# kelaendi/mused

Hardware: AMD Instinct MI355X
Metric: stream rows/sec, d=1024 l=128 window=10k synthetic (SWFD + kNN similarity + eigenstep + labels) (higher is better)
Workload: dtype f64; 1 GPU; synthetic d=1024 l=128 window=10000 k=50 (BASELINE config 2); stream=blob, W=10000, d=1024, l=128, k=50, modalities=1, swfd_levels=14, rccl_ranks=1, lanes_per_gpu=20, padded_window_slots=2

## Files before the change

### mused_amd/csrc/gemm_f64.h

```cpp
#pragma once
#include <cstdlib>
#include <mutex>
#include <type_traits>
#include "internal.h"

namespace mused {

typedef double v4f64 __attribute__((ext_vector_type(4)));

constexpr int GEMM_BM = 128;
constexpr int GEMM_BN = 128;
constexpr int GEMM_BK = 16;
constexpr int GEMM_LD = 144;
constexpr int GEMM_THREADS = 256;
constexpr int GEMM_LDS_BYTES = 2  * 2  * GEMM_BK * GEMM_LD * 8;

struct GemmArgs {
  const void* A;
  const void* B;
  long lda, ldb;
  long strideA, strideB;
  int M, N, K;
  int kchunk;
  int splitk;
  int bsplit;
  int tiles_m, tiles_n;
  const int* rep;
  const int* list;
  const int* kact;
  int sym;
  const double* tail;
  long tail_stride;
  int tail_per;
  const int* tail_split;
  int tail_split_stride;
  int tail_pend;
  const double* tail_zero;
};

struct GemmSplit {
  const double* tail;
  const double* zero;
  int nk, nend;
};
__device__ __forceinline__ const double* split_row(const double* __restrict__ base, long ld, const GemmSplit& sp, int r, int nrows,
                                                   bool& zero) {
  zero = r >= sp.nend || r >= nrows;
  return zero ? sp.zero : (r < sp.nk ? base + (long)r * ld : sp.tail + (long)(r - sp.nk) * ld);
}

template <typename TIn, bool VEC>
__device__ __forceinline__ void stage_load_kc(const TIn* __restrict__ src, long ld, int r0, int nrows, int k0,
                                              int kend, TIn (&r)[8]) {
  const int m = threadIdx.x & 127;
  const int kh = threadIdx.x >> 7;
  const int row = r0 + m;
  const int k = k0 + kh * 8;
  if (row < nrows) {
    const TIn* p = src + (long)row * ld + k;
    if (VEC && k + 8 <= kend) {
      if (sizeof(TIn) == 4) {
        const float4 a = *reinterpret_cast<const float4*>(p);
        const float4 b = *reinterpret_cast<const float4*>(p + 4);
        r[0] = a.x; r[1] = a.y; r[2] = a.z; r[3] = a.w;
        r[4] = b.x; r[5] = b.y; r[6] = b.z; r[7] = b.w;
      } else {
        const double2* q = reinterpret_cast<const double2*>(p);
#pragma unroll
        for (int j = 0; j < 4; ++j) {
          const double2 v = q[j];
// ... 361 lines not shown
    diag_mirror_groups<W, GI + 1>(g, epi, z, m0, patch, acc);
  }
}

template <int W, int N, typename Epi>
__device__ __forceinline__ void diag_store_blocks(const GemmArgs& g, const Epi& epi, int z, int m0, const v4f64 (&acc)[9]) {
  if constexpr (N < 9) {
    const int lane = threadIdx.x & 63;
    const int col = m0 + DIAG_J[W][N] * 16 + (lane & 15);
#pragma unroll
    for (int r = 0; r < 4; ++r) {
      const int row = m0 + DIAG_I[W][N] * 16 + (lane >> 4) + 4 * r;
      if (row < g.M && col < g.N) epi(z, row, col, acc[N][r]);
    }
    diag_store_blocks<W, N + 1>(g, epi, z, m0, acc);
  }
}

template <int W, typename Epi>
__device__ __forceinline__ void diag_epilogue(const GemmArgs& g, const Epi& epi, int z, int m0, double* smem,
                                              const v4f64 (&acc)[9]) {
  diag_store_blocks<W, 0>(g, epi, z, m0, acc);
  diag_mirror_groups<W, 0>(g, epi, z, m0, smem + W * (16 * DIAG_PATCH_LD), acc);
}

inline int gemm_sym_diag_enabled() {
  static const int on = [] {
    const char* s = getenv("MUSED_GEMM_SYM_DIAG");
    return (s && s[0] == '0') ? 0 : 1;
  }();
  return on;
}

template <typename TA, typename TB, bool A_KC, bool B_KC, bool VEC, typename Epi, bool TAIL = false>
__global__ __launch_bounds__(GEMM_THREADS, 2) void gemm_f64_kernel(GemmArgs g, Epi epi) {
  extern __shared__ __attribute__((aligned(16))) double smem[];

  int z = blockIdx.z;
  int zb = g.bsplit ? z / g.bsplit : z;
  if (g.list) {
    if (zb >= g.list[0]) return;
    const int e = g.list[1 + zb];
    z += (e - zb) * (g.bsplit ? g.bsplit : 1);
    zb = e;
  } else if (g.rep && g.rep[zb] != zb) return;
  int tm, tn;
  if (g.sym) {
    const int t = g.tiles_n, nwg = t * (t + 1) / 2;
    const int e = xcd_remap(blockIdx.x, nwg);
    int r = (int)((2.0 * t + 1.0 - sqrt((2.0 * t + 1.0) * (2.0 * t + 1.0) - 8.0 * e)) * 0.5);
    r = r < 0 ? 0 : (r > t - 1 ? t - 1 : r);
    while (r > 0 && r * t - r * (r - 1) / 2 > e) --r;
    while (r + 1 < t && (r + 1) * t - (r + 1) * r / 2 <= e) ++r;
    tm = r;
    tn = r + (e - (r * t - r * (r - 1) / 2));
  } else {
    const int nwg = g.tiles_m * g.tiles_n;
    const int wg = xcd_remap(blockIdx.x, nwg);
    constexpr int GROUP_M = 8;
    const int per_group = GROUP_M * g.tiles_n;
    const int group_id = wg / per_group;
    const int first_m = group_id * GROUP_M;
    const int group_size = min(g.tiles_m - first_m, GROUP_M);
    tm = first_m + (wg % group_size);
    tn = (wg % per_group) / group_size;
  }
  const int m0 = tm * GEMM_BM, n0 = tn * GEMM_BN;
  const bool mirror = g.sym && tm != tn;

  int k_lo = 0, k_hi = g.K;
  const TA* A = reinterpret_cast<const TA*>(g.A);
  const TB* B = reinterpret_cast<const TB*>(g.B);
  if (g.splitk) {
    k_lo = z * g.kchunk;
    k_hi = min(g.K, k_lo + g.kchunk);
  } else {
    A += (long)zb * g.strideA;
    B += (long)zb * g.strideB;
    if (g.bsplit) {
      k_lo = (z - zb * g.bsplit) * g.kchunk;
      k_hi = min(g.K, k_lo + g.kchunk);
    } else if (g.kact) {
      k_hi = min(g.K, g.kact[zb]);
    }
  }

  GemmSplit sp{};
  if constexpr (TAIL) {
    sp.nk = g.tail_split[(long)zb * g.tail_split_stride];
    sp.nend = sp.nk + g.tail_pend;
    sp.tail = g.tail + (long)(zb / g.tail_per) * g.tail_stride;
    sp.zero = g.tail_zero;
  }

  if constexpr (std::is_same<TA, TB>::value && A_KC == B_KC) {
    if (g.sym == 2 && tm == tn) {
      const int w = __builtin_amdgcn_readfirstlane(threadIdx.x >> 6);
      v4f64 acc9[9];
      gemm_tile_mainloop_diag<TA, A_KC, VEC, TAIL>(g, A, m0, k_lo, k_hi, smem, w, acc9, sp);
      switch (w) {
        case 0: diag_epilogue<0>(g, epi, z, m0, smem, acc9); break;
        case 1: diag_epilogue<1>(g, epi, z, m0, smem, acc9); break;
        case 2: diag_epilogue<2>(g, epi, z, m0, smem, acc9); break;
        default: diag_epilogue<3>(g, epi, z, m0, smem, acc9); break;
      }
      return;
    }
  }

  const int lane = threadIdx.x & 63;
  const int wave = threadIdx.x >> 6;
  const int wr = wave >> 1, wc = wave & 1;
  const int kq = lane >> 4, li = lane & 15;

  v4f64 acc[4][4];
  gemm_tile_mainloop<TA, TB, A_KC, B_KC, VEC, TAIL>(g, A, B, m0, n0, k_lo, k_hi, smem, acc, sp);

#pragma unroll
  for (int i = 0; i < 4; ++i) {
#pragma unroll
    for (int j = 0; j < 4; ++j) {
      const int col = n0 + wc * 64 + j * 16 + li;
#pragma unroll
      for (int r = 0; r < 4; ++r) {
        const int row = m0 + wr * 64 + i * 16 + kq + 4 * r;
// ... 13 lines not shown
          const int j = half * 2 + jj;
          const int col = n0 + wc * 64 + j * 16 + li;
#pragma unroll
          for (int r = 0; r < 4; ++r) {
            const int rl = i * 16 + kq + 4 * r;
            const int rg = m0 + wr * 64 + rl;
            patch[(jj * 16 + li) * 65 + rl] = (rg < g.M && col < g.N) ? epi.value(col, rg, acc[i][j][r]) : 0.0;
          }
        }
      const int rowm = m0 + wr * 64 + lane;
#pragma unroll 8
      for (int c = 0; c < 32; ++c) {
        const int colm = n0 + wc * 64 + half * 32 + c;
        if (colm < g.N && rowm < g.M) epi.put(z, colm, rowm, patch[c * 65 + lane]);
      }
    }
  }
}

struct EpiStore {
  double* C;
  long ldc;
  long strideC;
  double alpha;
  __device__ __forceinline__ void operator()(int z, int row, int col, double v) const {
    C[(long)z * strideC + (long)row * ldc + col] = alpha * v;
  }
  __device__ __forceinline__ double value(int, int, double v) const { return alpha * v; }
  __device__ __forceinline__ void put(int z, int row, int col, double val) const {
    C[(long)z * strideC + (long)row * ldc + col] = val;
  }
};

template <typename TA, typename TB, bool A_KC, bool B_KC, bool VEC, typename Epi, bool TAIL = false>
int gemm_f64_prepare_t() {
  static LdsOptIn opt;
  auto k = gemm_f64_kernel<TA, TB, A_KC, B_KC, VEC, Epi, TAIL>;
  const hipError_t err = allow_dynamic_lds(opt, reinterpret_cast<const void*>(k), GEMM_LDS_BYTES);
  MUSED_CHECK_HIP(err);
  return MUSED_OK;
}

template <typename TA, typename TB, bool A_KC, bool B_KC, typename Epi, bool TAIL = false>
int gemm_f64_launch_t(GemmArgs g, int batch, Epi epi, bool vec, hipStream_t stream) {
  g.tiles_m = cdiv(g.M, GEMM_BM);
  g.tiles_n = cdiv(g.N, GEMM_BN);
  if (g.sym) g.sym = (g.sym != 3 && gemm_sym_diag_enabled()) ? 2 : 1;
  if (g.M <= 0 || g.N <= 0 || batch <= 0) return MUSED_OK;
  dim3 grid(g.sym ? g.tiles_n * (g.tiles_n + 1) / 2 : g.tiles_m * g.tiles_n, 1, batch);
  int rc;
  if (vec) {
    if ((rc = gemm_f64_prepare_t<TA, TB, A_KC, B_KC, true, Epi, TAIL>())) return rc;
    hipLaunchKernelGGL((gemm_f64_kernel<TA, TB, A_KC, B_KC, true, Epi, TAIL>), grid, dim3(GEMM_THREADS), GEMM_LDS_BYTES,
                       stream, g, epi);
  } else {
    if ((rc = gemm_f64_prepare_t<TA, TB, A_KC, B_KC, false, Epi, TAIL>())) return rc;
    hipLaunchKernelGGL((gemm_f64_kernel<TA, TB, A_KC, B_KC, false, Epi, TAIL>), grid, dim3(GEMM_THREADS), GEMM_LDS_BYTES,
                       stream, g, epi);
  }
  MUSED_LAUNCH_CHECK();
  return MUSED_OK;
}

template <typename T>
static inline bool vec_ok(const void* p, long ld, long stride) {
  const long e = 16 / (long)sizeof(T);
  return ((uintptr_t)p % 16 == 0) && (ld % e == 0) && (stride % e == 0);
}

}
```

### mused_amd/csrc/gemm_f64.hip

```cpp
#include <stdarg.h>

#include "gemm_f64.h"
#include "internal.h"

namespace mused {

static thread_local char g_err[512] = "";

void set_error(const char* fmt, ...) {
  va_list ap;
  va_start(ap, fmt);
  vsnprintf(g_err, sizeof(g_err), fmt, ap);
  va_end(ap);
}

const char* last_error() { return g_err; }

int gemm_f64_prepare_all() {
  int rc = 0;
#define PREP(a, b, v) rc |= gemm_f64_prepare_t<double, double, a, b, v, EpiStore>()
  PREP(true, true, true); PREP(true, true, false); PREP(true, false, true); PREP(true, false, false);
  PREP(false, true, true); PREP(false, true, false); PREP(false, false, true); PREP(false, false, false);
#undef PREP
#define PREP(a, b, v) rc |= gemm_f64_prepare_t<double, double, a, b, v, EpiStore, true>()
  PREP(true, true, true); PREP(true, true, false); PREP(true, false, true); PREP(true, false, false);
#undef PREP
  return rc ? MUSED_ERR_HIP : MUSED_OK;
}

static int gemm_set_tail(GemmArgs& g, const GemmTail& t, bool a_kc, bool b_kc, long ld, bool& vec) {
  MUSED_REQUIRE(t.rows && t.split && t.zero_row && t.per_lane >= 1 && t.pend >= 0, "gemm_f64: bad tail");
  MUSED_REQUIRE(a_kc && (!b_kc || g.sym), "gemm_f64: a tail needs a Gram launch or a K-rows operand B");
  g.tail = t.rows; g.tail_stride = t.lane_stride; g.tail_per = t.per_lane;
  g.tail_split = t.split; g.tail_split_stride = t.split_stride; g.tail_pend = t.pend; g.tail_zero = t.zero_row;
  if (g.sym && t.plain_diag) g.sym = 3;
  vec = vec && vec_ok<double>(t.rows, ld, t.lane_stride) && vec_ok<double>(t.zero_row, ld, 0);
  return MUSED_OK;
}

int gemm_f64(bool a_kc, bool b_kc, const double* A, long lda, long strideA, const double* B, long ldb,
             long strideB, double* C, long ldc, long strideC, int M, int N, int K, int batch, double alpha,
             hipStream_t stream, const int* rep, const int* list, const int* kact, const GemmTail* tail) {
  GemmArgs g;
  memset(&g, 0, sizeof(g));
  g.A = A; g.B = B; g.lda = lda; g.ldb = ldb; g.strideA = strideA; g.strideB = strideB;
  g.M = M; g.N = N; g.K = K; g.splitk = 0; g.kchunk = 0;
  g.rep = rep; g.list = list; g.kact = kact;
  g.sym = (A == B && a_kc == b_kc && lda == ldb && strideA == strideB && M == N) ? 1 : 0;
  EpiStore epi{C, ldc, strideC, alpha};
  bool vec = vec_ok<double>(A, lda, strideA) && vec_ok<double>(B, ldb, strideB);
  if (tail) {
    int rc;
    if ((rc = gemm_set_tail(g, *tail, a_kc, b_kc, ldb, vec))) return rc;
    if (b_kc) return gemm_f64_launch_t<double, double, true, true, EpiStore, true>(g, batch, epi, vec, stream);
    return gemm_f64_launch_t<double, double, true, false, EpiStore, true>(g, batch, epi, vec, stream);
  }
  if (a_kc && b_kc) return gemm_f64_launch_t<double, double, true, true>(g, batch, epi, vec, stream);
  if (a_kc && !b_kc) return gemm_f64_launch_t<double, double, true, false>(g, batch, epi, vec, stream);
  if (!a_kc && b_kc) return gemm_f64_launch_t<double, double, false, true>(g, batch, epi, vec, stream);
  return gemm_f64_launch_t<double, double, false, false>(g, batch, epi, vec, stream);
}

int gemm_f64_splitk(bool a_kc, bool b_kc, const double* A, long lda, const double* B, long ldb, double* partial,
                    int M, int N, int K, int kchunk, int nsplit, hipStream_t stream) {
  MUSED_REQUIRE(kchunk > 0 && kchunk % GEMM_BK == 0 && nsplit >= 1 && (long)kchunk * nsplit >= K,
                "gemm_f64_splitk: bad kchunk %d x %d for K=%d", kchunk, nsplit, K);
  GemmArgs g;
  memset(&g, 0, sizeof(g));
  g.A = A; g.B = B; g.lda = lda; g.ldb = ldb;
  g.M = M; g.N = N; g.K = K; g.splitk = 1; g.kchunk = kchunk;
  EpiStore epi{partial, (long)N, (long)M * N, 1.0};
  const bool vec = vec_ok<double>(A, lda, 0) && vec_ok<double>(B, ldb, 0);
  if (a_kc && b_kc) return gemm_f64_launch_t<double, double, true, true>(g, nsplit, epi, vec, stream);
  if (a_kc && !b_kc) return gemm_f64_launch_t<double, double, true, false>(g, nsplit, epi, vec, stream);
  if (!a_kc && b_kc) return gemm_f64_launch_t<double, double, false, true>(g, nsplit, epi, vec, stream);
  return gemm_f64_launch_t<double, double, false, false>(g, nsplit, epi, vec, stream);
}

__global__ void splitk_reduce_kernel(const double* __restrict__ partial, int nsplit, long count,
                                     double* __restrict__ out) {
  const long i = (long)blockIdx.x * blockDim.x + threadIdx.x;
  if (i >= count) return;
  double s = 0.0;
  for (int z = 0; z < nsplit; ++z) s += partial[(long)z * count + i];
  out[i] = s;
}

int gemm_f64_batched_splitk(bool a_kc, bool b_kc, const double* A, long lda, long strideA, const double* B, long ldb, long strideB,
                            double* partial, int M, int N, int K, int batch, int kchunk, int nsplit, hipStream_t stream,
                            const int* rep, const int* list, const GemmTail* tail) {
  MUSED_REQUIRE(kchunk > 0 && kchunk % GEMM_BK == 0 && nsplit >= 1 && (long)kchunk * nsplit >= K,
                "gemm_f64_batched_splitk: bad kchunk %d x %d for K=%d", kchunk, nsplit, K);
  GemmArgs g;
// ... 75 lines not shown

int mused_gemm_f64_batched_rep(int a_kc, int b_kc, const double* A, long lda, long strideA, const double* B, long ldb,
                               long strideB, double* C, long ldc, long strideC, int M, int N, int K, int batch,
                               double alpha, const int* rep, void* stream) {
  return mused::gemm_f64(a_kc != 0, b_kc != 0, A, lda, strideA, B, ldb, strideB, C, ldc, strideC, M, N, K, batch,
                         alpha, (hipStream_t)stream, rep);
}

int mused_debug_gemm_f64_batched_active(int a_kc, int b_kc, const double* A, long lda, long strideA, const double* B, long ldb,
                                        long strideB, double* C, long ldc, long strideC, int M, int N, int K, int batch,
                                        double alpha, const int* list, const int* kact, void* stream) {
  return mused::gemm_f64(a_kc != 0, b_kc != 0, A, lda, strideA, B, ldb, strideB, C, ldc, strideC, M, N, K, batch,
                         alpha, (hipStream_t)stream, nullptr, list, kact);
}

int mused_debug_gemm_f64_batched_tail(int a_kc, int b_kc, const double* A, long lda, long strideA, const double* B, long ldb,
                                      long strideB, double* C, long ldc, long strideC, int M, int N, int K, int batch,
                                      const int* list, const int* kact, const double* tail, long tail_stride, int per_lane,
                                      const int* split, int split_stride, int pend, const double* zero_row, int plain_diag, double* partial,
                                      int kchunk,
                                      int nsplit, void* stream) {
  MUSED_REQUIRE(A && B && C && tail && split && batch >= 1, "mused_debug_gemm_f64_batched_tail: bad arguments");
  const mused::GemmTail t{tail, tail_stride, per_lane, split, split_stride, pend, zero_row, plain_diag};
  if (nsplit <= 1)
    return mused::gemm_f64(a_kc != 0, b_kc != 0, A, lda, strideA, B, ldb, strideB, C, ldc, strideC, M, N, K, batch, 1.0,
                           (hipStream_t)stream, nullptr, list, kact, &t);
  MUSED_REQUIRE(partial && ldc == N && strideC == (long)M * N, "mused_debug_gemm_f64_batched_tail: split-K writes a dense C");
  int rc = mused::gemm_f64_batched_splitk(a_kc != 0, b_kc != 0, A, lda, strideA, B, ldb, strideB, partial, M, N, K, batch, kchunk,
                                          nsplit, (hipStream_t)stream, nullptr, list, &t);
  if (rc != MUSED_OK) return rc;
  return mused::gemm_batched_splitk_reduce(partial, nsplit, (long)M * N, C, batch, nullptr, (hipStream_t)stream, list);
}

int mused_gemm_f64_splitk(int a_kc, int b_kc, const double* A, long lda, const double* B, long ldb, double* partial,
                          double* C, int M, int N, int K, int kchunk, int nsplit, void* stream) {
  MUSED_REQUIRE(A && B && partial && C && M >= 0 && N >= 0 && K >= 0, "mused_gemm_f64_splitk: bad arguments");
  int rc = mused::gemm_f64_splitk(a_kc != 0, b_kc != 0, A, lda, B, ldb, partial, M, N, K, kchunk, nsplit,
                                  (hipStream_t)stream);
  if (rc != MUSED_OK || M == 0 || N == 0) return rc;
  return mused::gemm_splitk_reduce(partial, nsplit, (long)M * N, C, (hipStream_t)stream);
}

int mused_gemm_f64_batched_splitk(int a_kc, int b_kc, const double* A, long lda, long strideA, const double* B, long ldb,
                                  long strideB, double* partial, double* C, int M, int N, int K, int batch, int kchunk,
                                  int nsplit, const int* rep, void* stream) {
  MUSED_REQUIRE(A && B && partial && C && M >= 0 && N >= 0 && K >= 0 && batch >= 1,
                "mused_gemm_f64_batched_splitk: bad arguments");
  int rc = mused::gemm_f64_batched_splitk(a_kc != 0, b_kc != 0, A, lda, strideA, B, ldb, strideB, partial, M, N, K, batch,
                                          kchunk, nsplit, (hipStream_t)stream, rep);
  if (rc != MUSED_OK || M == 0 || N == 0) return rc;
  return mused::gemm_batched_splitk_reduce(partial, nsplit, (long)M * N, C, batch, rep, (hipStream_t)stream);
}

}
```

### mused_amd/csrc/internal.h

```cpp
#pragma once
#include "common.h"

#include <atomic>
#include <mutex>

extern "C" int mused_row_sq_norms(const void* X, int dtype, long n, int d, long ld, double* out, void* stream);

namespace mused {

int select_from_records(const double* rec, int n, int kind, int k, int* out_idx, unsigned long long* out_mask,
                        int mask_words, hipStream_t stream);
int select_from_tag_sets(const int* rowptr, const int* tags, const int* postptr, const int* postrow, int n, int k,
                         int* out_idx, unsigned long long* out_mask, int mask_words, hipStream_t stream);
int select_max_fused_rows(bool tag_sets);
int select_window_records(const double* rec, const int* vrank, int s, int e, int kind, int k, unsigned long long* out_mask,
                          int mask_words, hipStream_t stream);
int select_window_tag_sets(const int* rowptr, const int* tags, const int* postptr, const int* postrow, const int* vrank, int s,
                           int e, int k, unsigned long long* out_mask, int mask_words, hipStream_t stream);

std::recursive_mutex& capture_mutex();
using CaptureLock = std::lock_guard<std::recursive_mutex>;

struct LdsOptIn {
  std::atomic<bool> done{false};
  hipError_t err = hipSuccess;
};
inline hipError_t allow_dynamic_lds(LdsOptIn& s, const void* kernel, size_t bytes) {
  if (!s.done.load(std::memory_order_acquire)) {
    CaptureLock lock(capture_mutex());
    if (!s.done.load(std::memory_order_relaxed)) {
      s.err = hipFuncSetAttribute(kernel, hipFuncAttributeMaxDynamicSharedMemorySize, (int)bytes);
      s.done.store(true, std::memory_order_release);
    }
  }
  return s.err;
}
inline hipError_t allow_dynamic_lds(hipError_t before, LdsOptIn& s, const void* kernel, size_t bytes) {
  return before != hipSuccess ? before : allow_dynamic_lds(s, kernel, bytes);
}


struct GemmTail {
  const double* rows;
  long lane_stride;
  int per_lane;
  const int* split;
  int split_stride;
  int pend;
  const double* zero_row;
  int plain_diag;
};
int gemm_f64(bool a_kc, bool b_kc, const double* A, long lda, long strideA, const double* B, long ldb,
             long strideB, double* C, long ldc, long strideC, int M, int N, int K, int batch, double alpha,
             hipStream_t stream, const int* rep = nullptr, const int* list = nullptr, const int* kact = nullptr,
             const GemmTail* tail = nullptr);

int gemm_f64_batched_splitk(bool a_kc, bool b_kc, const double* A, long lda, long strideA, const double* B, long ldb, long strideB,
                            double* partial, int M, int N, int K, int batch, int kchunk, int nsplit, hipStream_t stream,
                            const int* rep = nullptr, const int* list = nullptr, const GemmTail* tail = nullptr);
int gemm_batched_splitk_reduce(const double* partial, int nsplit, long count, double* out, int batch, const int* rep,
                               hipStream_t stream, const int* list = nullptr);
int gemm_f64_prepare_all();

int gemm_f64_splitk(bool a_kc, bool b_kc, const double* A, long lda, const double* B, long ldb, double* partial,
                    int M, int N, int K, int kchunk, int nsplit, hipStream_t stream);
int gemm_splitk_reduce(const double* partial, int nsplit, long count, double* out, hipStream_t stream);

int lu_permute_l(double* Y, int n, int r, long ld, int* pivstep, double* prow, long ws_f64_len, hipStream_t st);
int qr_economic(double* Y, int n, int r, long ldy, double* Q, long ldq, double* tau, double* wpart, hipStream_t st,
                const int* run_if = nullptr);
int spmm_binary(const int* rowptr, const int* colidx, int n, const double* Q, long ldq, int r, double* Y, long ldy,
                hipStream_t stream, const double* col_sign = nullptr);

int spmm_valued(const int* rowptr, const int* colidx, const double* vals, int n, const double* Q, long ldq, int r, double* Y,
                long ldy, hipStream_t stream, const double* col_sign = nullptr);

constexpr int ADJ_VAL_MAX_M = 8;
struct AdjValSrc {
  const void* p[ADJ_VAL_MAX_M];
  double w[ADJ_VAL_MAX_M];
  long ld;
  int M, dtype;
};
int adj_val_src_masks(const unsigned long long* const* masks, const double* weights, int M, AdjValSrc* out, const char* who);
int adj_val_src_dense(const void* dense, int dtype, int n, long ld, AdjValSrc* out, const char* who);
int adj_val_src_store(const AdjValSrc& src, AdjValSrc* dst, hipStream_t st);
int adj_csr_values_dev(const AdjValSrc* src_dev, bool dense, int n, int words, const int* rowptr, const int* colidx,
                       int transposed, double* vals, int* flag, hipStream_t st);
// ... 52 lines not shown
```

### mused_amd/csrc/swfd.hip

```cpp
#include <vector>

#include "internal.h"

namespace mused {

struct Swfd {
  int N, d, ell, L, S, cap, n2, n4, n3;
  int lanes;
  double R;
  long i;
  int pend;
  long restart_mark;
  int skip_dead;
  bool twin;
  int sweeps;
  double* buf;
  double* pendbuf;
  bool shared;
  int* froze;
  int* nk0;
  bool tail_dirty;
  bool settle;
  int* used;
  double* queue;
  long long* qt;
  int* meta;
  int* rep;
  int* list;
  int* offs;
  int oround;
  int* kact;
  long long* ostat;
  long long* dropped;
  double* theta;
  double *T, *Wc;
  int gram_split;
  double* gpart;
  int* plan;
  int* keep_src;
  long long* now_dev;
  int* status;
  int* status_host;
  EigPlan* eig;
  double *stack, *Wq, *Bout, *sig_out, *qinfo;
  int* qsel;
  EigPlan* eigq;
  EigPlan* eigq3;
  int pre_chunk;
  double *pre_in, *pre_out, *pre_gram;
  EigPlan* eigp;
};

static inline int sk_index(const Swfd* h, int lane, int level, int kind) { return lane * 2 * h->L + kind * h->L + level; }

struct BitWord { unsigned long long w; };
template <typename T>
__device__ __forceinline__ double row_elem(const T* row, int c) { return (double)row[c]; }
template <>
__device__ __forceinline__ double row_elem<BitWord>(const BitWord* row, int c) {
  return (double)((row[c >> 6].w >> (c & 63)) & 1ull);
}

template <typename T>
__device__ __forceinline__ double2 row_pair(const T* row, int c);
template <>
__device__ __forceinline__ double2 row_pair<double>(const double* row, int c) { return *(const double2*)(row + c); }
template <>
__device__ __forceinline__ double2 row_pair<long long>(const long long* row, int c) {
  const longlong2 v = *(const longlong2*)(row + c);
  return make_double2((double)v.x, (double)v.y);
}
template <>
__device__ __forceinline__ double2 row_pair<float>(const float* row, int c) {
  const float2 v = *(const float2*)(row + c);
  return make_double2((double)v.x, (double)v.y);
}
template <>
__device__ __forceinline__ double2 row_pair<BitWord>(const BitWord* row, int c) {
  const unsigned long long w = row[c >> 6].w >> (c & 63);
  return make_double2((double)(w & 1ull), (double)((w >> 1) & 1ull));
}
template <typename T> struct RowPairAlign { static constexpr unsigned long long mask = 15; };
template <> struct RowPairAlign<float> { static constexpr unsigned long long mask = 7; };
// ... 307 lines not shown
template <typename Src>
__global__ void swfd_settle_shared_kernel(const double* __restrict__ T, const int* __restrict__ plan,
                                          const int* __restrict__ keep_src, const int* __restrict__ meta,
                                          const int* __restrict__ froze, int fill_all, double* __restrict__ buf,
                                          double* __restrict__ queue, double* __restrict__ pendbuf, int n2, int ell, int cap, int d,
                                          const int* __restrict__ rep, const Src* __restrict__ X, long ldx, long lane_stride,
                                          int per_lane, int nxt, int pend0) {
  const int rho = blockIdx.x, s = blockIdx.y;
  const int lane = s / per_lane;
  const int sr = rep ? rep[s] : s;
  const int nk = meta[s * 4 + 0];
  if (s == lane * per_lane && rho < nxt)
    row_copy<Src>(pendbuf + ((long)lane * ell + rho) * d, X + (long)lane * lane_stride + (long)rho * ldx, d);
  if (sr < 0) {
    if (nk + rho >= n2) return;
    double* dst = buf + ((long)s * n2 + nk + rho) * d;
    if (rho < nxt) {
      row_copy<Src>(dst, X + (long)lane * lane_stride + (long)rho * ldx, d);
    } else if (froze[s]) {
      if (rho < pend0) row_copy<double>(dst, pendbuf + ((long)lane * ell + rho) * d, d);
      else if (!fill_all) row_zero(dst, d);
    }
    return;
  }
  const double* Ts = T + (long)sr * ell * d;
  if (rho < ell && plan[(s * ell + rho) * 2] == 2) {
    const int slot = plan[(s * ell + rho) * 2 + 1];
    row_copy<double>(queue + ((long)s * cap + slot) * d, Ts + (long)rho * d, d);
  }
  if (rho < nk) row_copy<double>(buf + ((long)s * n2 + rho) * d, Ts + (long)keep_src[s * ell + rho] * d, d);
}

template <typename Src>
static int swfd_rotate_all(Swfd* h, hipStream_t st, const Src* next, long ldx, long lane_stride, int nxt) {
  const int S = h->S, n2 = h->n2, d = h->d, ell = h->ell;
  int rc;
  if (h->rep)
    hipLaunchKernelGGL(swfd_rep_kernel, dim3(1), dim3(1024), sizeof(int) * (size_t)S, st, h->meta, h->L, 2 * h->lanes, h->rep,
                       h->twin ? 1 : 0, h->dropped, (long long)(((h->i - 1) / h->N) * h->N), h->skip_dead, h->now_dev,
                       (long long)h->i, h->pend, ell, n2, h->list, h->offs, h->kact, h->ostat, h->oround, h->froze);
  else
    hipLaunchKernelGGL(swfd_set_now_kernel, dim3(1), dim3(1), 0, st, h->now_dev, (long long)h->i);
  const GemmTail gram_tail{h->pendbuf, (long)ell * d, 2 * h->L, h->meta, 4, h->pend, h->pendbuf + (long)h->lanes * ell * d, 0};
  const GemmTail rot_tail{h->pendbuf, (long)ell * d, 2 * h->L, h->nk0, 1, h->pend, h->pendbuf + (long)h->lanes * ell * d, 0};
  if (h->gram_split > 1) {
    const int kchunk = ((d + h->gram_split - 1) / h->gram_split + 15) / 16 * 16;
    if ((rc = gemm_f64_batched_splitk(true, true, h->buf, d, (long)n2 * d, h->buf, d, (long)n2 * d, h->gpart, n2, n2, d, S, kchunk,
                                      h->gram_split, st, h->rep, h->list, h->shared ? &gram_tail : nullptr)))
      return rc;
    if ((rc = gemm_batched_splitk_reduce(h->gpart, h->gram_split, (long)n2 * n2, eig_plan_input(h->eig), S, h->rep, st, h->list)))
      return rc;
  } else if ((rc = gemm_f64(true, true, h->buf, d, (long)n2 * d, h->buf, d, (long)n2 * d, eig_plan_input(h->eig), n2,
                            (long)n2 * n2, n2, n2, d, S, 1.0, st, h->rep, h->list, nullptr, h->shared ? &gram_tail : nullptr)))
    return rc;
  if ((rc = eig_plan_run_inplace(h->eig, nullptr, nullptr, st, true))) return rc;
  const EigColumns e = eig_plan_columns(h->eig);
  hipLaunchKernelGGL(swfd_decide_kernel, dim3(S), dim3(1024), 0, st, e.lam, e.cols, e.ld, n2, ell, h->cap, h->N, h->now_dev,
                     h->theta, h->meta, h->qt, h->dropped, h->plan, h->keep_src, h->Wc, h->rep, h->settle ? h->used : nullptr,
                     h->pend, h->nk0);
  if ((rc = gemm_f64(true, false, h->Wc, n2, (long)ell * n2, h->buf, d, (long)n2 * d, h->T, d, (long)ell * d, ell, d,
                     n2, S, 1.0, st, h->rep, h->list, h->kact, h->shared ? &rot_tail : nullptr)))
    return rc;
  if (h->shared) {
    hipLaunchKernelGGL(swfd_settle_shared_kernel<Src>, dim3(n2, S), dim3(256), 0, st, h->T, h->plan, h->keep_src, h->meta,
                       h->froze, h->tail_dirty ? 1 : 0, h->buf, h->queue, h->pendbuf, n2, ell, h->cap, d, h->rep, next, ldx,
                       lane_stride, 2 * h->L, nxt, h->pend);
    h->tail_dirty = false;
  } else if (h->settle) {
    hipLaunchKernelGGL(swfd_settle_kernel<Src>, dim3(n2, S), dim3(256), 0, st, h->T, h->plan, h->keep_src, h->meta, h->used,
                       h->tail_dirty ? 1 : 0, h->buf, h->queue, n2, ell, h->cap, d, h->rep, next, ldx, lane_stride, 2 * h->L,
                       nxt);
    h->tail_dirty = false;
  } else {
    hipLaunchKernelGGL(swfd_scatter_kernel, dim3(n2, S), dim3(256), 0, st, h->T, h->plan, h->keep_src, h->meta, h->buf,
                       h->queue, n2, ell, h->cap, d, h->rep);
  }
// ... 41 lines not shown
  if (col < ell) v = (row < ell) ? gram[z * ell * ell + (long)col * ell + row] : ((row - ell == col) ? 1.0 : 0.0);
  Gc[z * n2 * n2 + e] = v;
}

template <typename T>
static int swfd_prerotate(Swfd* h, const T* X, long ldx, long lane_stride, const PreBlocks& pb, int nblk, hipStream_t st) {
  const int ell = h->ell, d = h->d, B = h->lanes, n2 = h->n2;
  int rc;
  const int Z = nblk * B;
  hipLaunchKernelGGL(swfd_pre_load_kernel<T>, dim3(ell, Z), dim3(256), 0, st, X, ldx, lane_stride, B, ell, d, pb,
                     h->pre_in);
  if ((rc = gemm_f64(true, true, h->pre_in, d, (long)ell * d, h->pre_in, d, (long)ell * d, h->pre_gram, ell,
                     (long)ell * ell, ell, ell, d, Z, 1.0, st)))
    return rc;
  hipLaunchKernelGGL(swfd_pre_pack_kernel, dim3(cdiv((long)n2 * n2, 256), Z), dim3(256), 0, st, h->pre_gram, ell,
                     eig_plan_input(h->eigp));
  if ((rc = eig_plan_run_inplace(h->eigp, nullptr, nullptr, st, true))) return rc;
  const double* cols = eig_plan_columns(h->eigp).cols;
  const int ld = eig_plan_columns(h->eigp).ld;
  if ((rc = gemm_f64(true, false, cols + ell, ld, (long)ld * ld, h->pre_in, d, (long)ell * d, h->pre_out, d, (long)ell * d,
                     ell, d, ell, Z, 1.0, st)))
    return rc;
  MUSED_LAUNCH_CHECK();
  return MUSED_OK;
}

template <typename T>
static int swfd_append_t(Swfd* h, const T* X, long ldx, long lane_stride, long m, hipStream_t st) {
  long r = 0;
  int rc;
  PreBlocks pb;
  int pre_n = 0, pre_next = 0;
  int placed = 0;
  while (r < m) {
    if (h->i > 0 && h->i % h->N == 0 && h->restart_mark != h->i) {
      if ((rc = swfd_restart(h, st))) return rc;
      h->restart_mark = h->i;
      h->twin = false;
    }
    const long in_epoch = h->i % h->N;
    long until = h->ell - (in_epoch % h->ell);
    if (h->N - in_epoch < until) until = h->N - in_epoch;
    const long take = (m - r) < until ? (m - r) : until;
    bool from_pre = false;
    if (h->pre_chunk > 0 && h->pend == 0 && take == until) {
      if (pre_next >= pre_n) {
        pre_n = pre_next = 0;
        long rr = r, ii = h->i;
        while (pre_n < h->pre_chunk && rr < m) {
          const long ie = ii % h->N;
          long u = h->ell - (ie % h->ell);
          if (h->N - ie < u) u = h->N - ie;
          if (m - rr < u) break;
          pb.row0[pre_n] = (int)rr;
          pb.rows[pre_n] = (int)u;
          ++pre_n;
          rr += u;
          ii += u;
        }
        if ((rc = swfd_prerotate<T>(h, X, ldx, lane_stride, pb, pre_n, st))) return rc;
      }
      from_pre = true;
    }
    if (placed > 0) {
      if (placed != take) {
        set_error("mused_swfd_append: internal: %d rows placed ahead, the block takes %ld", placed, take);
        return MUSED_ERR_STATE;
      }
      placed = 0;
    } else if (from_pre) {
      const double* src = h->pre_out + (long)pre_next * h->lanes * h->ell * h->d;
      hipLaunchKernelGGL(swfd_append_kernel<double>, dim3((int)take, h->S), dim3(256), 0, st, src, (long)h->d,
                         (long)h->ell * h->d, 2 * h->L, (int)take, h->d, h->n2, h->pend, h->meta, h->buf);
      ++pre_next;
    } else if (h->shared) {
      hipLaunchKernelGGL(swfd_append_shared_kernel<T>, dim3((int)take, h->S), dim3(256), 0, st, X + r * ldx, ldx, lane_stride,
                         2 * h->L, (int)take, h->d, h->n2, h->ell, h->pend, h->meta, h->rep, h->buf, h->pendbuf);
    } else {
      hipLaunchKernelGGL(swfd_append_kernel<T>, dim3((int)take, h->S), dim3(256), 0, st, X + r * ldx, ldx, lane_stride,
                         2 * h->L, (int)take, h->d, h->n2, h->pend, h->meta, h->buf);
    }
    MUSED_LAUNCH_CHECK();
    h->pend += (int)take;
    h->i += take;
    r += take;
    if (take == until) {
      long nxt = 0;
      if (h->settle && h->pre_chunk == 0 && r < m && h->i % h->N != 0) {
        const long ie = h->i % h->N;
        long u = h->ell - (ie % h->ell);
        if (h->N - ie < u) u = h->N - ie;
        nxt = (m - r) < u ? (m - r) : u;
      }
      if ((rc = swfd_rotate_all<T>(h, st, nxt ? X + r * ldx : nullptr, ldx, lane_stride, (int)nxt))) return rc;
      placed = (int)nxt;
    }
  }
  return MUSED_OK;
}

__global__ void swfd_select_kernel(const int* __restrict__ meta, const long long* __restrict__ qt,
                                   const long long* __restrict__ dropped, int L, int cap, int N, long long now,
                                   int* __restrict__ qsel_all) {
  if (threadIdx.x != 0) return;
  const int lane = blockIdx.x;
  const int base = lane * 2 * L;
  int* qsel = qsel_all + (long)lane * (4 + cap);
  int lvl = L - 1;
  for (int j = 0; j < L; ++j) {
    const long long dr = dropped[base + j];
    if (dr == 0 || dr + N <= now) { lvl = j; break; }
  }
  const int sk = base + lvl;
  const int head = meta[sk * 4 + 1], cnt = meta[sk * 4 + 2];
  int ns = 0;
  for (int q = 0; q < cnt; ++q) {
    const int slot = (head + q) % cap;
    if (qt[(long)sk * cap + slot] + N > now) qsel[4 + ns++] = slot;
  }
  qsel[0] = lvl;
  qsel[1] = ns;
  qsel[2] = meta[sk * 4 + 0];
  qsel[3] = sk;
}

__global__ void swfd_stack_kernel(const int* __restrict__ qsel_all, const double* __restrict__ buf,
                                  const double* __restrict__ queue, int n2, int n4, int cap, int d, int pend,
// ... 246 lines not shown
  if ((rc = gemm_f64_prepare_all())) return rc;
  if ((rc = eig_plan_create(h->n2, h->S, h->sweeps, true, &h->eig, h->rep, EIG_PLAN_TOP_HALF, h->status, 0, h->list, h->offs)))
    return rc;
  if ((rc = eig_plan_create(h->n4, lanes, h->sweeps + 2, true, &h->eigq, nullptr, EIG_PLAN_TOP_FD, h->status, ell))) return rc;
  if (h->n3 < h->n4 &&
      (rc = eig_plan_create(h->n3, lanes, h->sweeps + 2, true, &h->eigq3, nullptr, EIG_PLAN_TOP_FD, h->status, ell)))
    return rc;
  {
    const char* pr = getenv("MUSED_SWFD_PREROT");
    const bool want_pre = pr ? (pr[0] != '0') : !eig_plan_direct_solver(h->eig);
    if (want_pre) {
      const size_t per_block = (size_t)lanes * ell * dd * 8;
      size_t c = ((size_t)256 << 20) / per_block;
      c = c < 1 ? 1 : (c > (size_t)SWFD_PRE_MAX ? (size_t)SWFD_PRE_MAX : c);
      h->pre_chunk = (int)c;
      MUSED_CHECK_HIP(hipMalloc((void**)&h->pre_in, c * per_block));
      MUSED_CHECK_HIP(hipMalloc((void**)&h->pre_out, c * per_block));
      MUSED_CHECK_HIP(hipMalloc((void**)&h->pre_gram, 8 * c * lanes * l * l));
      const char* ps = getenv("MUSED_SWFD_PREROT_SWEEPS");
      const int psw = ps ? atoi(ps) : 5;
      if ((rc = eig_plan_create(h->n2, (int)c * lanes, psw > 0 ? psw : 5, true, &h->eigp, nullptr,
                                EIG_PLAN_FIXED_SWEEPS | EIG_PLAN_NO_SORT, h->status)))
        return rc;
    }
  }
  {
    const char* sh = getenv("MUSED_SWFD_SHARED");
    h->shared = h->settle && h->pre_chunk == 0 && !(sh && sh[0] == '0');
    if (!h->shared) {
      (void)hipFree(h->froze); h->froze = nullptr;
      (void)hipFree(h->nk0); h->nk0 = nullptr;
    }
  }
  return MUSED_OK;
}

int mused_swfd_destroy(void* handle) {
  Swfd* h = (Swfd*)handle;
  if (!h) return MUSED_OK;
  CaptureLock resource_guard(capture_mutex());
  eig_plan_destroy(h->eig);
  eig_plan_destroy(h->eigq);
  if (h->eigq3) eig_plan_destroy(h->eigq3);
  if (h->eigp) eig_plan_destroy(h->eigp);
  void* bufs[] = {h->buf, h->queue, h->qt, h->meta, h->dropped, h->theta, h->T, h->Wc, h->plan,
                  h->keep_src, h->now_dev, h->stack, h->Wq, h->Bout, h->sig_out, h->qinfo, h->qsel,
                  h->rep, h->pre_in, h->pre_out, h->pre_gram, h->status, h->gpart, h->list, h->offs, h->kact, h->ostat, h->used,
                  h->pendbuf, h->froze, h->nk0};
  for (void* b : bufs) (void)hipFree(b);
  if (h->status_host) (void)hipHostFree(h->status_host);
  delete h;
  return MUSED_OK;
}

int mused_swfd_levels(void* handle) { return handle ? ((Swfd*)handle)->L : -1; }

int mused_swfd_profile(void* handle, int on) {
  Swfd* h = (Swfd*)handle;
  MUSED_REQUIRE(h, "mused_swfd_profile: null handle");
  return eig_plan_profile(h->eig, on != 0);
}

int mused_swfd_profile_read(void* handle, double* total_ms, long* launches, double* bytes_per_launch) {
  Swfd* h = (Swfd*)handle;
  MUSED_REQUIRE(h && total_ms && launches && bytes_per_launch, "mused_swfd_profile_read: null pointer");
  return eig_plan_profile_read(h->eig, total_ms, launches, bytes_per_launch);
}

extern "C" int mused_swfd_profile_read_direct(void* handle, double* total_ms, long* launches, double* matrices_solved,
                                              int* direct, double* tridiag_ms) {
  Swfd* h = (Swfd*)handle;
  MUSED_REQUIRE(h && total_ms && launches && matrices_solved && direct, "mused_swfd_profile_read_direct: null pointer");
  *direct = eig_plan_direct_solver(h->eig) ? 1 : 0;
  return eig_plan_profile_read_direct(h->eig, total_ms, launches, matrices_solved, tridiag_ms);
}

int mused_swfd_append_lanes(void* handle, const void* rows, int dtype, long n_rows, long ld, long lane_stride,
                            void* stream);

int mused_swfd_append(void* handle, const void* rows, int dtype, long n_rows, long ld, void* stream) {
  Swfd* h = (Swfd*)handle;
// ... 7 lines not shown
  MUSED_REQUIRE(h && (rows || n_rows == 0) && n_rows >= 0, "mused_swfd_append: bad arguments");
  hipStream_t st = (hipStream_t)stream;
  if (dtype == MUSED_BITS) {
    MUSED_REQUIRE(ld >= (h->d + 63) / 64, "mused_swfd_append: bit rows need a pitch of at least ceil(d / 64) words");
    return swfd_append_t<BitWord>(h, (const BitWord*)rows, ld, lane_stride, n_rows, st);
  }
  MUSED_REQUIRE(ld >= h->d, "mused_swfd_append: row pitch smaller than d");
  if (dtype == MUSED_F32) return swfd_append_t<float>(h, (const float*)rows, ld, lane_stride, n_rows, st);
  if (dtype == MUSED_F64) return swfd_append_t<double>(h, (const double*)rows, ld, lane_stride, n_rows, st);
  if (dtype == MUSED_I64) return swfd_append_t<long long>(h, (const long long*)rows, ld, lane_stride, n_rows, st);
  set_error("mused_swfd_append: unsupported dtype %d", dtype);
  return MUSED_ERR_UNSUPPORTED;
}

int mused_swfd_lanes(void* handle) { return handle ? ((Swfd*)handle)->lanes : -1; }

int mused_swfd_debug_state(void* handle, int* rep_out, int* meta_out) {
  Swfd* h = (Swfd*)handle;
  if (!h) return MUSED_ERR_ARG;
  MUSED_CHECK_HIP(hipDeviceSynchronize());
  if (h->rep && rep_out) MUSED_CHECK_HIP(hipMemcpy(rep_out, h->rep, 4 * (size_t)h->S, hipMemcpyDeviceToHost));
  if (meta_out) MUSED_CHECK_HIP(hipMemcpy(meta_out, h->meta, 16 * (size_t)h->S, hipMemcpyDeviceToHost));
  return h->rep ? 1 : 0;
}

int mused_swfd_debug_used(void* handle, int* used_out) {
  Swfd* h = (Swfd*)handle;
  if (!h || !used_out) return MUSED_ERR_ARG;
  if (!h->used) return 0;
  MUSED_CHECK_HIP(hipDeviceSynchronize());
  MUSED_CHECK_HIP(hipMemcpy(used_out, h->used, 4 * (size_t)h->S, hipMemcpyDeviceToHost));
  return 1;
}

int mused_swfd_debug_shared(void* handle) { return handle ? (((Swfd*)handle)->shared ? 1 : 0) : MUSED_ERR_ARG; }

int mused_swfd_debug_orders(void* handle, long long* out) {
  Swfd* h = (Swfd*)handle;
  if (!h || !out) return MUSED_ERR_ARG;
  if (!h->ostat) return 0;
  MUSED_CHECK_HIP(hipDeviceSynchronize());
  MUSED_CHECK_HIP(hipMemcpy(out, h->ostat, 8 * 18, hipMemcpyDeviceToHost));
  return 1;
}

int mused_swfd_query(void* handle, double* out_sketch, double* out_sigma, double* out_info, void* stream) {
  Swfd* h = (Swfd*)handle;
  MUSED_REQUIRE(h && out_sketch, "mused_swfd_query: null pointer");
  return swfd_query(h, out_sketch, out_sigma, out_info, (hipStream_t)stream);
}

int mused_swfd_status(void* handle, int* status_out, void* stream) {
  Swfd* h = (Swfd*)handle;
  MUSED_REQUIRE(h && status_out, "mused_swfd_status: null pointer");
  MUSED_CHECK_HIP(hipMemcpyAsync(h->status_host, h->status, sizeof(int), hipMemcpyDeviceToHost, (hipStream_t)stream));
  MUSED_CHECK_HIP(hipStreamSynchronize((hipStream_t)stream));
  *status_out = *h->status_host;
  return MUSED_OK;
}

int mused_swfd_counters(void* handle, long* rows_seen, int* pending) {
  Swfd* h = (Swfd*)handle;
  MUSED_REQUIRE(h && rows_seen && pending, "mused_swfd_counters: null pointer");
  *rows_seen = h->i;
  *pending = h->pend;
  return MUSED_OK;
// ... 100 lines not shown
```

Baseline: 663,800 rows/s.

## Precompute pending-row Gram blocks in chunks and fill them into SWFD Gram tiles

Adds a grouped Gram GEMM that computes the l×l Gram of each incoming row block for several upcoming epochs and all lanes in one batched launch. The per-rotation Gram GEMM then copies these precomputed values into tiles that lie entirely in the pending-row region, instead of recomputing them from the tail buffer. The aim is fewer, larger launches and less redundant K=d work per rotation. The cost is an extra 32MB-class buffer and a new launch path. It is enabled by default when n2 > 128 under the shared, non-split configuration.

```diff
diff --git a/mused_amd/csrc/gemm_f64.h b/mused_amd/csrc/gemm_f64.h
--- a/mused_amd/csrc/gemm_f64.h
+++ b/mused_amd/csrc/gemm_f64.h
@@ -36,6 +36,11 @@
   int tail_split_stride;
   int tail_pend;
   const double* tail_zero;
+  const double* fill;
+  long fill_stride;
+  int fill_ld;
+  int grp_per;
+  long grp_stride;
 };
 
 struct GemmSplit {
@@ -463,7 +468,21 @@
   return on;
 }
 
-template <typename TA, typename TB, bool A_KC, bool B_KC, bool VEC, typename Epi, bool TAIL = false>
+template <typename Epi>
+__device__ __forceinline__ void gemm_fill_tile(const GemmArgs& g, const Epi& epi, int z, const double* __restrict__ pp, int nk,
+                                               int nend, int r0, int c0) {
+  const int c = c0 + (threadIdx.x & 127);
+  if (c >= g.N) return;
+  const bool cin = c < nend;
+  const int rlim = min(g.M, r0 + GEMM_BM);
+#pragma unroll 8
+  for (int r = r0 + (threadIdx.x >> 7); r < rlim; r += 2) {
+    const double v = (cin && r < nend) ? pp[(long)(r - nk) * g.fill_ld + (c - nk)] : 0.0;
+    epi.put(z, r, c, epi.value(r, c, v));
+  }
+}
+
+template <typename TA, typename TB, bool A_KC, bool B_KC, bool VEC, typename Epi, bool TAIL = false, bool GRP = false>
 __global__ __launch_bounds__(GEMM_THREADS, 2) void gemm_f64_kernel(GemmArgs g, Epi epi) {
   extern __shared__ __attribute__((aligned(16))) double smem[];
 
@@ -506,8 +525,14 @@
     k_lo = z * g.kchunk;
     k_hi = min(g.K, k_lo + g.kchunk);
   } else {
-    A += (long)zb * g.strideA;
-    B += (long)zb * g.strideB;
+    if constexpr (GRP) {
+      const int grp = zb / g.grp_per;
+      A += (long)(zb - grp * g.grp_per) * g.strideA + (long)grp * g.grp_stride;
+      B += (long)(zb - grp * g.grp_per) * g.strideB + (long)grp * g.grp_stride;
+    } else {
+      A += (long)zb * g.strideA;
+      B += (long)zb * g.strideB;
+    }
     if (g.bsplit) {
       k_lo = (z - zb * g.bsplit) * g.kchunk;
       k_hi = min(g.K, k_lo + g.kchunk);
@@ -522,6 +547,14 @@
     sp.nend = sp.nk + g.tail_pend;
     sp.tail = g.tail + (long)(zb / g.tail_per) * g.tail_stride;
     sp.zero = g.tail_zero;
+    if constexpr (A_KC && B_KC) {
+      if (g.fill && g.sym && m0 >= sp.nk) {
+        const double* pp = g.fill + (long)(zb / g.tail_per) * g.fill_stride;
+        gemm_fill_tile(g, epi, z, pp, sp.nk, sp.nend, m0, n0);
+        if (mirror) gemm_fill_tile(g, epi, z, pp, sp.nk, sp.nend, n0, m0);
+        return;
+      }
+    }
   }
 
   if constexpr (std::is_same<TA, TB>::value && A_KC == B_KC) {
@@ -601,16 +634,16 @@
   }
 };
 
-template <typename TA, typename TB, bool A_KC, bool B_KC, bool VEC, typename Epi, bool TAIL = false>
+template <typename TA, typename TB, bool A_KC, bool B_KC, bool VEC, typename Epi, bool TAIL = false, bool GRP = false>
 int gemm_f64_prepare_t() {
   static LdsOptIn opt;
-  auto k = gemm_f64_kernel<TA, TB, A_KC, B_KC, VEC, Epi, TAIL>;
+  auto k = gemm_f64_kernel<TA, TB, A_KC, B_KC, VEC, Epi, TAIL, GRP>;
   const hipError_t err = allow_dynamic_lds(opt, reinterpret_cast<const void*>(k), GEMM_LDS_BYTES);
   MUSED_CHECK_HIP(err);
   return MUSED_OK;
 }
 
-template <typename TA, typename TB, bool A_KC, bool B_KC, typename Epi, bool TAIL = false>
+template <typename TA, typename TB, bool A_KC, bool B_KC, typename Epi, bool TAIL = false, bool GRP = false>
 int gemm_f64_launch_t(GemmArgs g, int batch, Epi epi, bool vec, hipStream_t stream) {
   g.tiles_m = cdiv(g.M, GEMM_BM);
   g.tiles_n = cdiv(g.N, GEMM_BN);
@@ -619,12 +652,12 @@
   dim3 grid(g.sym ? g.tiles_n * (g.tiles_n + 1) / 2 : g.tiles_m * g.tiles_n, 1, batch);
   int rc;
   if (vec) {
-    if ((rc = gemm_f64_prepare_t<TA, TB, A_KC, B_KC, true, Epi, TAIL>())) return rc;
-    hipLaunchKernelGGL((gemm_f64_kernel<TA, TB, A_KC, B_KC, true, Epi, TAIL>), grid, dim3(GEMM_THREADS), GEMM_LDS_BYTES,
+    if ((rc = gemm_f64_prepare_t<TA, TB, A_KC, B_KC, true, Epi, TAIL, GRP>())) return rc;
+    hipLaunchKernelGGL((gemm_f64_kernel<TA, TB, A_KC, B_KC, true, Epi, TAIL, GRP>), grid, dim3(GEMM_THREADS), GEMM_LDS_BYTES,
                        stream, g, epi);
   } else {
-    if ((rc = gemm_f64_prepare_t<TA, TB, A_KC, B_KC, false, Epi, TAIL>())) return rc;
-    hipLaunchKernelGGL((gemm_f64_kernel<TA, TB, A_KC, B_KC, false, Epi, TAIL>), grid, dim3(GEMM_THREADS), GEMM_LDS_BYTES,
+    if ((rc = gemm_f64_prepare_t<TA, TB, A_KC, B_KC, false, Epi, TAIL, GRP>())) return rc;
+    hipLaunchKernelGGL((gemm_f64_kernel<TA, TB, A_KC, B_KC, false, Epi, TAIL, GRP>), grid, dim3(GEMM_THREADS), GEMM_LDS_BYTES,
                        stream, g, epi);
   }
   MUSED_LAUNCH_CHECK();
diff --git a/mused_amd/csrc/gemm_f64.hip b/mused_amd/csrc/gemm_f64.hip
--- a/mused_amd/csrc/gemm_f64.hip
+++ b/mused_amd/csrc/gemm_f64.hip
@@ -25,6 +25,10 @@
 #define PREP(a, b, v) rc |= gemm_f64_prepare_t<double, double, a, b, v, EpiStore, true>()
   PREP(true, true, true); PREP(true, true, false); PREP(true, false, true); PREP(true, false, false);
 #undef PREP
+  rc |= gemm_f64_prepare_t<double, double, true, true, true, EpiStore, false, true>();
+  rc |= gemm_f64_prepare_t<double, double, true, true, false, EpiStore, false, true>();
+  rc |= gemm_f64_prepare_t<float, float, true, true, true, EpiStore, false, true>();
+  rc |= gemm_f64_prepare_t<float, float, true, true, false, EpiStore, false, true>();
   return rc ? MUSED_ERR_HIP : MUSED_OK;
 }
 
@@ -34,6 +38,10 @@
   g.tail = t.rows; g.tail_stride = t.lane_stride; g.tail_per = t.per_lane;
   g.tail_split = t.split; g.tail_split_stride = t.split_stride; g.tail_pend = t.pend; g.tail_zero = t.zero_row;
   if (g.sym && t.plain_diag) g.sym = 3;
+  if (t.fill) {
+    MUSED_REQUIRE(g.sym && !g.bsplit && !g.splitk && t.fill_ld >= t.pend, "gemm_f64: a fill source needs a Gram launch that is not split over K");
+    g.fill = t.fill; g.fill_stride = t.fill_stride; g.fill_ld = t.fill_ld;
+  }
   vec = vec && vec_ok<double>(t.rows, ld, t.lane_stride) && vec_ok<double>(t.zero_row, ld, 0);
   return MUSED_OK;
 }
@@ -59,6 +67,24 @@
   if (a_kc && !b_kc) return gemm_f64_launch_t<double, double, true, false>(g, batch, epi, vec, stream);
   if (!a_kc && b_kc) return gemm_f64_launch_t<double, double, false, true>(g, batch, epi, vec, stream);
   return gemm_f64_launch_t<double, double, false, false>(g, batch, epi, vec, stream);
+}
+
+int gemm_gram_rows(const void* A, bool f32, long lda, long strideA, int per_group, long group_stride, double* C, long ldc,
+                   long strideC, int M, int K, int batch, int plain_diag, hipStream_t stream) {
+  MUSED_REQUIRE(per_group >= 1 && ldc >= M, "gemm_gram_rows: bad arguments");
+  GemmArgs g;
+  memset(&g, 0, sizeof(g));
+  g.A = A; g.B = A; g.lda = lda; g.ldb = lda; g.strideA = strideA; g.strideB = strideA;
+  g.M = M; g.N = M; g.K = K;
+  g.sym = plain_diag ? 3 : 1;
+  g.grp_per = per_group; g.grp_stride = group_stride;
+  EpiStore epi{C, ldc, strideC, 1.0};
+  if (f32) {
+    const bool vec = vec_ok<float>(A, lda, strideA) && group_stride % 4 == 0;
+    return gemm_f64_launch_t<float, float, true, true, EpiStore, false, true>(g, batch, epi, vec, stream);
+  }
+  const bool vec = vec_ok<double>(A, lda, strideA) && group_stride % 2 == 0;
+  return gemm_f64_launch_t<double, double, true, true, EpiStore, false, true>(g, batch, epi, vec, stream);
 }
 
 int gemm_f64_splitk(bool a_kc, bool b_kc, const double* A, long lda, const double* B, long ldb, double* partial,
@@ -200,6 +226,23 @@
   return mused::gemm_batched_splitk_reduce(partial, nsplit, (long)M * N, C, batch, nullptr, (hipStream_t)stream, list);
 }
 
+int mused_debug_gemm_f64_batched_tail_fill(const double* A, long lda, long strideA, double* C, long ldc, long strideC, int n, int K,
+                                           int batch, const int* list, const double* tail, long tail_stride, int per_lane,
+                                           const int* split, int split_stride, int pend, const double* zero_row, int plain_diag,
+                                           const double* fill, long fill_stride, int fill_ld, void* stream) {
+  MUSED_REQUIRE(A && C && tail && split && fill && batch >= 1, "mused_debug_gemm_f64_batched_tail_fill: bad arguments");
+  const mused::GemmTail t{tail, tail_stride, per_lane, split, split_stride, pend, zero_row, plain_diag, fill, fill_stride, fill_ld};
+  return mused::gemm_f64(true, true, A, lda, strideA, A, lda, strideA, C, ldc, strideC, n, n, K, batch, 1.0, (hipStream_t)stream,
+                         nullptr, list, nullptr, &t);
+}
+
+int mused_debug_gemm_gram_rows(const void* A, int dtype, long lda, long strideA, int per_group, long group_stride, double* C,
+                               long ldc, long strideC, int M, int K, int batch, int plain_diag, void* stream) {
+  MUSED_REQUIRE(A && C && batch >= 1 && (dtype == MUSED_F32 || dtype == MUSED_F64), "mused_debug_gemm_gram_rows: bad arguments");
+  return mused::gemm_gram_rows(A, dtype == MUSED_F32, lda, strideA, per_group, group_stride, C, ldc, strideC, M, K, batch,
+                               plain_diag, (hipStream_t)stream);
+}
+
 int mused_gemm_f64_splitk(int a_kc, int b_kc, const double* A, long lda, const double* B, long ldb, double* partial,
                           double* C, int M, int N, int K, int kchunk, int nsplit, void* stream) {
   MUSED_REQUIRE(A && B && partial && C && M >= 0 && N >= 0 && K >= 0, "mused_gemm_f64_splitk: bad arguments");
diff --git a/mused_amd/csrc/internal.h b/mused_amd/csrc/internal.h
--- a/mused_amd/csrc/internal.h
+++ b/mused_amd/csrc/internal.h
@@ -49,11 +49,16 @@
   int pend;
   const double* zero_row;
   int plain_diag;
+  const double* fill;
+  long fill_stride;
+  int fill_ld;
 };
 int gemm_f64(bool a_kc, bool b_kc, const double* A, long lda, long strideA, const double* B, long ldb,
              long strideB, double* C, long ldc, long strideC, int M, int N, int K, int batch, double alpha,
              hipStream_t stream, const int* rep = nullptr, const int* list = nullptr, const int* kact = nullptr,
              const GemmTail* tail = nullptr);
+int gemm_gram_rows(const void* A, bool f32, long lda, long strideA, int per_group, long group_stride, double* C, long ldc,
+                   long strideC, int M, int K, int batch, int plain_diag, hipStream_t stream);
 
 int gemm_f64_batched_splitk(bool a_kc, bool b_kc, const double* A, long lda, long strideA, const double* B, long ldb, long strideB,
                             double* partial, int M, int N, int K, int batch, int kchunk, int nsplit, hipStream_t stream,
diff --git a/mused_amd/csrc/swfd.hip b/mused_amd/csrc/swfd.hip
--- a/mused_amd/csrc/swfd.hip
+++ b/mused_amd/csrc/swfd.hip
@@ -1,3 +1,4 @@
+#include <type_traits>
 #include <vector>
 
 #include "internal.h"
@@ -49,6 +50,8 @@
   int pre_chunk;
   double *pre_in, *pre_out, *pre_gram;
   EigPlan* eigp;
+  int ppt_chunk;
+  double* ppt;
 };
 
 static inline int sk_index(const Swfd* h, int lane, int level, int kind) { return lane * 2 * h->L + kind * h->L + level; }
@@ -422,7 +425,8 @@
 }
 
 template <typename Src>
-static int swfd_rotate_all(Swfd* h, hipStream_t st, const Src* next, long ldx, long lane_stride, int nxt) {
+static int swfd_rotate_all(Swfd* h, hipStream_t st, const Src* next, long ldx, long lane_stride, int nxt,
+                           const double* ppt = nullptr) {
   const int S = h->S, n2 = h->n2, d = h->d, ell = h->ell;
   int rc;
   if (h->rep)
@@ -431,7 +435,8 @@
                        (long long)h->i, h->pend, ell, n2, h->list, h->offs, h->kact, h->ostat, h->oround, h->froze);
   else
     hipLaunchKernelGGL(swfd_set_now_kernel, dim3(1), dim3(1), 0, st, h->now_dev, (long long)h->i);
-  const GemmTail gram_tail{h->pendbuf, (long)ell * d, 2 * h->L, h->meta, 4, h->pend, h->pendbuf + (long)h->lanes * ell * d, 0};
+  const GemmTail gram_tail{h->pendbuf, (long)ell * d, 2 * h->L, h->meta, 4, h->pend, h->pendbuf + (long)h->lanes * ell * d, 0,
+                           ppt, (long)ell * ell, ell};
   const GemmTail rot_tail{h->pendbuf, (long)ell * d, 2 * h->L, h->nk0, 1, h->pend, h->pendbuf + (long)h->lanes * ell * d, 0};
   if (h->gram_split > 1) {
     const int kchunk = ((d + h->gram_split - 1) / h->gram_split + 15) / 16 * 16;
@@ -539,6 +544,8 @@
   PreBlocks pb;
   int pre_n = 0, pre_next = 0;
   int placed = 0;
+  int ppt_n = 0, ppt_next = 0;
+  constexpr bool ppt_rows = std::is_same<T, float>::value || std::is_same<T, double>::value;
   while (r < m) {
     if (h->i > 0 && h->i % h->N == 0 && h->restart_mark != h->i) {
       if ((rc = swfd_restart(h, st))) return rc;
@@ -549,6 +556,27 @@
     long until = h->ell - (in_epoch % h->ell);
     if (h->N - in_epoch < until) until = h->N - in_epoch;
     const long take = (m - r) < until ? (m - r) : until;
+    const double* ppt = nullptr;
+    if (ppt_rows && h->ppt_chunk > 0 && h->pend == 0 && take == until) {
+      if (ppt_next >= ppt_n) {
+        ppt_n = ppt_next = 0;
+        long rr = r, ii = h->i;
+        while (ppt_n < h->ppt_chunk && rr < m) {
+          const long ie = ii % h->N;
+          long u = h->ell - (ie % h->ell);
+          if (h->N - ie < u) u = h->N - ie;
+          if (u != take || m - rr < u) break;
+          ++ppt_n;
+          rr += u;
+          ii += u;
+        }
+        if ((rc = gemm_gram_rows(X + r * ldx, std::is_same<T, float>::value, ldx, lane_stride, h->lanes, take * ldx, h->ppt,
+                                 h->ell, (long)h->ell * h->ell, (int)take, h->d, ppt_n * h->lanes, 0, st)))
+          return rc;
+      }
+      ppt = h->ppt + (long)ppt_next * h->lanes * h->ell * h->ell;
+      ++ppt_next;
+    }
     bool from_pre = false;
     if (h->pre_chunk > 0 && h->pend == 0 && take == until) {
       if (pre_next >= pre_n) {
@@ -599,7 +627,7 @@
         if (h->N - ie < u) u = h->N - ie;
         nxt = (m - r) < u ? (m - r) : u;
       }
-      if ((rc = swfd_rotate_all<T>(h, st, nxt ? X + r * ldx : nullptr, ldx, lane_stride, (int)nxt))) return rc;
+      if ((rc = swfd_rotate_all<T>(h, st, nxt ? X + r * ldx : nullptr, ldx, lane_stride, (int)nxt, ppt))) return rc;
       placed = (int)nxt;
     }
   }
@@ -912,6 +940,19 @@
       (void)hipFree(h->nk0); h->nk0 = nullptr;
     }
   }
+  {
+    const char* pp = getenv("MUSED_SWFD_PPT");
+    const size_t per_block = (size_t)lanes * ell * ell * 8;
+    size_t c = ((size_t)32 << 20) / per_block;
+    c = c > 16 ? 16 : c;
+    const char* pc = getenv("MUSED_SWFD_PPT_CHUNK");
+    if (pc && atoi(pc) >= 1 && (size_t)atoi(pc) < c) c = (size_t)atoi(pc);
+    const bool want = pp ? pp[0] != '0' : h->n2 > 128;
+    if (h->shared && h->gram_split == 1 && want && c >= 1) {
+      MUSED_CHECK_HIP(hipMalloc((void**)&h->ppt, c * per_block));
+      h->ppt_chunk = (int)c;
+    }
+  }
   return MUSED_OK;
 }
 
@@ -926,7 +967,7 @@
   void* bufs[] = {h->buf, h->queue, h->qt, h->meta, h->dropped, h->theta, h->T, h->Wc, h->plan,
                   h->keep_src, h->now_dev, h->stack, h->Wq, h->Bout, h->sig_out, h->qinfo, h->qsel,
                   h->rep, h->pre_in, h->pre_out, h->pre_gram, h->status, h->gpart, h->list, h->offs, h->kact, h->ostat, h->used,
-                  h->pendbuf, h->froze, h->nk0};
+                  h->pendbuf, h->froze, h->nk0, h->ppt};
   for (void* b : bufs) (void)hipFree(b);
   if (h->status_host) (void)hipHostFree(h->status_host);
   delete h;
@@ -1000,6 +1041,8 @@
   MUSED_CHECK_HIP(hipMemcpy(used_out, h->used, 4 * (size_t)h->S, hipMemcpyDeviceToHost));
   return 1;
 }
+
+int mused_swfd_debug_ppt(void* handle) { return handle ? ((Swfd*)handle)->ppt_chunk : MUSED_ERR_ARG; }
 
 int mused_swfd_debug_shared(void* handle) { return handle ? (((Swfd*)handle)->shared ? 1 : 0) : MUSED_ERR_ARG; }
 
```

Result: faster. 679,400 rows/s, median of 6 (+2.4%).
